# EmilDohne/compressed-image

Hardware: AMD Instinct MI355X
Metric: compress+decompress GB/s (uncompressed side) (higher is better)
Workload: dtype u8

## Files before the change

compressed-image_amd/csrc/encode_kernel.h:

```cpp
#pragma once
#include "codec_types.h"
#include "wave.h"
#include "decode_kernel.h"
#include "blosclz_kernel.h"
#include "zstd_encode.h"
#include "assemble_kernel.h"

namespace cimg {

struct EncodeArgs {
    const ChunkDesc* descs;
    int32_t nchunks;
    CodecParams p;
    const uint8_t* raw;
    uint8_t* scratch;
    StreamRec* recs;
    int32_t lds_bytes;
    int32_t total_blocks;
    int32_t want_split;
    uint64_t* dbg;
    uint32_t* queue;
    int32_t uniform_nblocks;
    int32_t block_items;
    uint32_t* zstd_seq;
    int32_t zstd_seq_stride;
    const ZstdEncTables* zstd_tables;
    uint32_t* queue_next;
    int32_t nwaves;
    int32_t assemble;
    uint8_t* comp;
    ChunkLayout* layout;
    ChunkLayout* layout_host;
    uint32_t* chunk_count;
    uint32_t* ready;
    int32_t* next_item;
    uint32_t gen;
    uint32_t* placed = nullptr;
    int32_t helpers = 0;
};

enum : int { ENC_NQ = 64, ENC_QSTRIDE = 32 };

enum : int { LZ4_HASH_BYTES = 16384, LZ4_MAX_INPUT_U16 = 65536 + 11 - 1 };

inline int encode_lds_bytes(int stream_bytes, int compcode = CODEC_LZ4)
{
    return compcode == CODEC_BLOSCLZ ? blz_encode_lds_bytes(stream_bytes) : round16(stream_bytes) + (compcode == CODEC_ZSTD ? (2 << ZSTD_ENC_HASH_BITS) : LZ4_HASH_BYTES);
}
CIMG_HD int encode_items(int total_blocks, int streams_per_block, bool split, int whole_blocks = 0)
{
    return split ? whole_blocks + (total_blocks - whole_blocks) * streams_per_block : total_blocks;
}
CIMG_HD bool encode_block_items_ok(int typesize, int filter, int blocksize)
{
    return (typesize == 2 || typesize == 4) && filter == FILTER_SHUFFLE && blocksize == 32768;
}

#if defined(CIMG_PROFILE) && !defined(CIMG_EMULATE)
#define CIMG_ITEM_STAMP(dbg, item, k) ((void)0)
#else
#define CIMG_ITEM_STAMP(dbg, item, k) debug_stamp(dbg, item, k)
#endif

#ifdef CIMG_EMULATE
extern long g_emu_windows, g_emu_matches, g_emu_collisions;
#define CIMG_STAT(x) (++(x))
#else
#define CIMG_STAT(x) ((void)0)
#endif

template <int HB = 13>
CIMG_DEV uint32_t lz4_hash(uint32_t v) { return (v * 2654435761u) >> (32 - HB); }
CIMG_DEV int skip_prefix(int n) { const int q = n >> 6, r = n & 63; return q * (32 * (q - 1) + r); }

CIMG_DEV void emit_len_ext(cimg_global_u8p out, int pos, int rem)
{
    const int n255 = rem / 255, last = rem - 255 * n255;
#ifndef CIMG_EMULATE
#pragma unroll 1
#endif
    for (int c = 0; c <= n255; c += 64) {
        FOR_LANES(l) { if (c + l <= n255) out[pos + c + l] = (uint8_t)(c + l < n255 ? 255 : last); }
    }
}

CIMG_DEV void emit_literals(const uint8_t* in, int from, cimg_global_u8p out, int pos, int count)
{
#ifndef CIMG_EMULATE
#pragma unroll 1
#endif
    for (int c = 0; c < count; c += 64) {
        FOR_LANES(l) { if (c + l < count) out[pos + c + l] = in[from + c + l]; }
    }
}

CIMG_DEV int match_more(const uint8_t* in, int ip, int mp, int maxc, int from, int n)
{
    int mcode = from;
    for (int it = 0; it <= n / 256 + 1; ++it) {
        LV<int> len;
        LV<bool> stop;
        FOR_LANES(l) {
            const int k = mcode + 4 * l;
            const uint32_t x = lds_ld32u(in, ip + 4 + k) ^ lds_ld32u(in, mp + 4 + k);
            const int ln = imin(x ? (int)(__builtin_ctz(x) >> 3) : 4, imax(maxc - k, 0));
            len[l] = ln;
            stop[l] = ln < 4;
        }
        const uint64_t sm = ballot(stop);
        if (sm) { const int f = ctz64(sm); return mcode + 4 * f + readlane(len, f); }
        mcode += 256;
    }
    return mcode;
}

CIMG_DEV int div255(int x) { return (int)(((uint64_t)(uint32_t)x * 0x80808081ull) >> 39); }

CIMG_DEV bool emit_pending(const uint8_t* in, cimg_global_u8p out, int cap, int& op, int& need, int np,
                           const LV<int>& P_anchor, const LV<int>& P_lit, const LV<int>& P_off, const LV<int>& P_mcode)
{
    LV<int> size, start, le, me;
    FOR_LANES(l) {
        const int lit = P_lit[l], mc = P_mcode[l];
        le[l] = lit >= 15 ? div255(lit - 15) + 1 : 0;
        me[l] = mc >= 15 ? div255(mc - 15) + 1 : 0;
        size[l] = l < np ? lit + 3 + le[l] + me[l] : 0;
    }
    int total;
    wave_exscan(size, start, total);
    LV<int> lhs, tokpos, litpos;
    LV<bool> fail, ext, shortlit, longlit;
    FOR_LANES(l) {
        const int lit = P_lit[l], mc = P_mcode[l];
        const bool act = l < np;
        tokpos[l] = op + start[l];
        litpos[l] = tokpos[l] + 1 + le[l];
        const int lhs1 = tokpos[l] + 1 + lit + 8 + div255(lit);
        const int lhs2 = litpos[l] + lit + 8 + div255(mc + 240);
        fail[l] = act && (lhs1 > cap || lhs2 > cap);
        lhs[l] = act ? imax(lhs1, lhs2) : 0;
        ext[l] = act && (le[l] > 0 || me[l] > 0);
        shortlit[l] = act && lit > 0 && lit <= 8;
        longlit[l] = act && lit > 8;
    }
    if (ballot(fail)) return false;
    need = imax(need, wave_max(lhs));
    FOR_LANES(l) {
        if (l < np) {
            const int lit = P_lit[l], mc = P_mcode[l], off = P_off[l];
            const int offpos = litpos[l] + lit;
            out[tokpos[l]] = (uint8_t)(((lit >= 15 ? 15 : lit) << 4) | (mc >= 15 ? 15 : mc));
            out[offpos] = (uint8_t)(off & 0xFF);
            out[offpos + 1] = (uint8_t)(off >> 8);
        }
    }
    if (ballot(ext)) {
        for (int r = 0; r < 4; ++r) {
            LV<bool> more;
            FOR_LANES(l) {
                const int lit = P_lit[l], mc = P_mcode[l];
                const bool act = l < np;
                const int le4 = le[l] <= 4 ? le[l] : 0, me4 = me[l] <= 4 ? me[l] : 0;
                if (act && r < le4) out[tokpos[l] + 1 + r] = (uint8_t)(r == le4 - 1 ? lit - 15 - 255 * (le4 - 1) : 255);
                if (act && r < me4) out[litpos[l] + lit + 2 + r] = (uint8_t)(r == me4 - 1 ? mc - 15 - 255 * (me4 - 1) : 255);
                more[l] = act && (r + 1 < le4 || r + 1 < me4);
            }
            if (!ballot(more)) break;
        }
        LV<bool> bigl, bigm;
        FOR_LANES(l) { bigl[l] = l < np && le[l] > 4; bigm[l] = l < np && me[l] > 4; }
        for (uint64_t m = ballot(bigl); m; m &= m - 1) {
            const int k = ctz64(m);
            emit_len_ext(out, readlane(tokpos, k) + 1, readlane(P_lit, k) - 15);
        }
        for (uint64_t m = ballot(bigm); m; m &= m - 1) {
            const int k = ctz64(m);
            emit_len_ext(out, readlane(litpos, k) + readlane(P_lit, k) + 2, readlane(P_mcode, k) - 15);
        }
    }
    if (ballot(shortlit)) {
        for (int r = 0; r < 8; ++r) {
            LV<bool> more;
            FOR_LANES(l) {
                if (shortlit[l] && r < P_lit[l]) out[litpos[l] + r] = in[P_anchor[l] + r];
                more[l] = shortlit[l] && r + 1 < P_lit[l];
            }
            if (!ballot(more)) break;
        }
    }
    uint64_t longm = ballot(longlit);
    while (longm) {
        const int k = ctz64(longm);
        longm &= longm - 1;
        emit_literals(in, readlane(P_anchor, k), out, readlane(litpos, k), readlane(P_lit, k));
    }
    op += total;
    return true;
}

template <int HB = 13>
CIMG_DEV bool lz4_no_match_at_all(const uint8_t* in, cimg_lds_vu16p tab16, int n, int s64, int f64, int mflimit_p1)
{
    bool verdict = false;
    for (int t0 = 0; t0 <= n; t0 += 64) {
        {
            LV<int> p1, p2;
            LV<bool> in2;
            FOR_LANES(l) {
                const int ta = t0 + l, tb = t0 + 64 + l;
                int pa = 1 + ta;
                if (ta > 0) pa = 2 + skip_prefix(s64 + ta - 1) - f64;
                const int pb = 2 + skip_prefix(s64 + tb - 1) - f64, gb = (s64 + tb - 1) >> 6;
                p1[l] = pa; p2[l] = pb;
                in2[l] = pb + gb <= mflimit_p1;
            }
            if (!~ballot(in2)) {
                LV<uint32_t> v1, v2, h1, h2, o1, o2, r1, r2, c1, c2;
                FOR_LANES(l) { v1[l] = lds_ld32u(in, p1[l]); v2[l] = lds_ld32u(in, p2[l]); h1[l] = lz4_hash<HB>(v1[l]); h2[l] = lz4_hash<HB>(v2[l]); }
                FOR_LANES(l) { o1[l] = tab16[h1[l]]; }
                FOR_LANES_W(l) { tab16[h1[l]] = (uint16_t)p1[l]; }
                FOR_LANES(l) { r1[l] = tab16[h1[l]]; }
                FOR_LANES(l) { o2[l] = tab16[h2[l]]; }
                FOR_LANES_W(l) { tab16[h2[l]] = (uint16_t)p2[l]; }
                FOR_LANES(l) { r2[l] = tab16[h2[l]]; c1[l] = lds_ld32u(in, (int)o1[l]); c2[l] = lds_ld32u(in, (int)o2[l]); }
                LV<bool> eventful;
                FOR_LANES(l) {
                    eventful[l] = (r1[l] != (uint32_t)(uint16_t)p1[l]) | (c1[l] == v1[l]) | (r2[l] != (uint32_t)(uint16_t)p2[l]) | (c2[l] == v2[l]);
                }
                if (!ballot(eventful)) { CIMG_STAT(g_emu_windows); CIMG_STAT(g_emu_windows); t0 += 64; continue; }
                FOR_LANES_W(l) { tab16[h2[l]] = (uint16_t)o2[l]; }
                FOR_LANES_W(l) { tab16[h1[l]] = (uint16_t)o1[l]; }
            }
        }
        LV<int> pos;
        LV<bool> inside;
        FOR_LANES(l) {
            const int t = t0 + l;
            int p = 1 + t, gap = 1;
            if (t > 0) { p = 2 + skip_prefix(s64 + t - 1) - f64; gap = (s64 + t - 1) >> 6; }
            pos[l] = p;
            inside[l] = p + gap <= mflimit_p1;
        }
        const uint64_t in_mask = ballot(inside);
        if (!in_mask) { verdict = true; break; }
        LV<uint32_t> v, h, old, rb, cv;
        LV<bool> lost, equal;
        FOR_LANES(l) { v[l] = lds_ld32u(in, inside[l] ? pos[l] : 0); h[l] = lz4_hash<HB>(v[l]); }
        FOR_LANES(l) { old[l] = tab16[h[l]]; }
        FOR_LANES_W(l) { if (inside[l]) tab16[h[l]] = (uint16_t)pos[l]; }
        FOR_LANES(l) { rb[l] = tab16[h[l]]; cv[l] = lds_ld32u(in, (int)old[l]); }
        FOR_LANES(l) {
            lost[l] = inside[l] & (rb[l] != (uint32_t)(uint16_t)pos[l]);
            equal[l] = inside[l] & (cv[l] == v[l]);
        }
        if (ballot(equal)) break;
        if (ballot(lost)) {
            LV<uint32_t> rb2, wv;
            LV<bool> crowd, same;
            FOR_LANES_W(l) { if (lost[l]) tab16[h[l]] = (uint16_t)pos[l]; }
            FOR_LANES(l) { rb2[l] = tab16[h[l]]; wv[l] = lds_ld32u(in, (int)rb[l]); }
            FOR_LANES(l) {
                crowd[l] = lost[l] & (rb2[l] != (uint32_t)(uint16_t)pos[l]);
                same[l] = lost[l] & (wv[l] == v[l]);
            }
            if (ballot(crowd) | ballot(same)) break;
            FOR_LANES_W(l) { if (inside[l] && rb2[l] != (uint32_t)(uint16_t)pos[l] && (uint32_t)pos[l] > rb2[l]) tab16[h[l]] = (uint16_t)pos[l]; }
        }
        CIMG_STAT(g_emu_windows);
        if (~in_mask) { verdict = true; break; }
    }
    return verdict;
}

template <bool SEQ = false>
CIMG_DEV int lz4_encode_body(const uint8_t* in, uint8_t* tab, int n, uint8_t* out_generic, int cap, int accel, int& need_out, uint64_t* dbg = nullptr, int item = 0, SeqSink* sink = nullptr)
{
    constexpr int HB = SEQ ? ZSTD_ENC_HASH_BITS : 13;
    cimg_global_u8p out = CIMG_AS_GLOBAL(out_generic);
    CIMG_PROF_DECL;
    (void)dbg; (void)item;

    cimg_lds_vu16p tab16 = CIMG_AS_LDS_VU16(tab);
    {
        const u128 z = {0, 0, 0, 0};
        for (int u0 = 0; u0 < (2 << HB) / 16; u0 += 64) {
            FOR_LANES(l) { st128a(tab + 16 * (u0 + l), z); }
        }
    }
    const int mflimit_p1 = n - 11, matchlimit = n - 5;
    const int s64 = accel << 6;
    const int f64 = skip_prefix(s64);
    int anchor = 0, op = 0, need = 0;
    LV<int> P_anchor, P_lit, P_off, P_mcode;
    int np = 0;
    FOR_LANES(l) { P_anchor[l] = 0; P_lit[l] = 0; P_off[l] = 0; P_mcode[l] = 0; }

    bool hopeless = false;
    if (n >= 13 + 64) {
        hopeless = lz4_no_match_at_all<HB>(in, tab16, n, s64, f64, mflimit_p1);
        if (hopeless) anchor = 0;
        else {
            const u128 z = {0, 0, 0, 0};
            for (int u0 = 0; u0 < (2 << HB) / 16; u0 += 64) {
                FOR_LANES(l) { st128a(tab + 16 * (u0 + l), z); }
            }
        }
    }
    if (n >= 13 && !hopeless) {
        {
            LV<uint32_t> v0;
            FOR_LANES(l) { v0[l] = lds_ld32u(in, 0); }
            FOR_LANES_W(l) { tab16[lz4_hash<HB>(v0[l])] = 0; }
        }
        CIMG_PROF_LAP(0);
        int sstart = 1;
        int t0 = 0;
        int pre = 0;
        LV<uint32_t> Wn;
        FOR_LANES(l) { Wn[l] = 0; }
        [[maybe_unused]] int chain_credit = 2;
        int guard = 0;
        int ending = 1;
        for (;;) {
            if (++guard > 2 * n + 4) { ending = -1; break; }
            LV<int> pos;
            LV<bool> valid;
            LV<uint32_t> v, h, back;
            int ip = 0, mp = 0, mcode = 0, backrun = 0;
            bool zero_lit = false;
            auto run_path = [&](const uint32_t v0, const uint32_t backv) {
                const int ip0 = sstart - 1;
                const uint32_t h0 = lz4_hash<HB>(v0);
                const uint32_t bbbb = (v0 & 0xFF) * 0x01010101u;
                FOR_LANES_W(l) { tab16[lz4_hash<HB>(backv)] = (uint16_t)(sstart - 3); }
                LV<uint32_t> slot, scan;
                LV<uint32_t> before;
                FOR_LANES(l) {
                    slot[l] = tab16[h0];
                    scan[l] = lds_ld32u(in, ip0 + 5 + 4 * l);
                    before[l] = in[ip0 - 1];
                }
                const int old0 = (int)readlane(slot, 0);
                LV<uint32_t> cw, iw;
                FOR_LANES(l) {
                    cw[l] = lds_ld32u(in, old0 + 4 * l);
                    iw[l] = lds_ld32u(in, ip0 + 4 * l);
                }
                needed_here(scan); needed_here(before); needed_here(iw);
                const bool hit0 = readlane(cw, 0) == v0;
                CIMG_STAT(g_emu_matches);
                if (hit0) {
                    CIMG_PROF_COUNT(5);
                    FOR_LANES_W(l) { tab16[h0] = (uint16_t)ip0; }
                    ip = ip0; mp = old0; zero_lit = true; backrun = 0;
                    const int maxc = matchlimit - (ip0 + 4);
                    LV<int> len;
                    LV<bool> stop;
                    FOR_LANES(l) {
                        const int k = 4 * (l - 1);
                        const uint32_t x = cw[l] ^ iw[l];
                        const int ln = imin(x ? (int)(__builtin_ctz(x) >> 3) : 4, imax(maxc - k, 0));
                        len[l] = ln;
                        stop[l] = (l >= 1) & (ln < 4);
                    }
                    const uint64_t sm = ballot(stop);
                    if (sm) { const int f = ctz64(sm); mcode = 4 * (f - 1) + readlane(len, f); }
                    else mcode = match_more(in, ip0, old0, maxc, 252, n);
                } else {
                    FOR_LANES_W(l) { tab16[h0] = (uint16_t)(ip0 + 1); }
                    ip = ip0 + 1; mp = ip0; zero_lit = false; mcode = 0;
                    backrun = (readlane(before, 0) == (v0 & 0xFF)) ? 1 : 0;
                    const int maxc = matchlimit - (ip + 4);
                    for (int scans = 0; scans <= n / 256 + 2; ++scans) {
                        LV<int> len;
                        LV<bool> stop;
                        FOR_LANES(l) {
                            const int k = mcode + 4 * l;
                            int vb = maxc - k;
                            vb = vb < 0 ? 0 : (vb > 4 ? 4 : vb);
                            int ln = 0;
                            if (vb > 0) {
                                const uint32_t x = scan[l] ^ bbbb;
                                ln = x ? (int)(__builtin_ctz(x) >> 3) : 4;
                                if (ln > vb) ln = vb;
                            }
                            len[l] = ln;
                            stop[l] = ln < 4;
                        }
                        const uint64_t sm = ballot(stop);
                        if (sm) { const int f = ctz64(sm); mcode += 4 * f + readlane(len, f); break; }
                        mcode += 256;
                        FOR_LANES(l) { scan[l] = lds_ld32u(in, ip + 4 + mcode + 4 * l); }
                    }
                }
            };
            const auto sequence = [&](auto extended_tag, int ip, int mp, int mcode, int backrun, const bool zero_lit) -> int {
            if constexpr (!decltype(extended_tag)::value) {
            CIMG_PROF_COUNT(3);
            const int room = zero_lit ? 0 : imin(ip - anchor, mp);
            const int maxc = matchlimit - (ip + 4);
                LV<bool> eq, stop;
                LV<int> len;
                FOR_LANES(l) {
                    const int kb = l < room ? l + 1 : 0;
                    const uint32_t pa = in[ip - kb], pb = in[mp - kb];
                    const int k = 4 * l;
                    const uint32_t x = lds_ld32u(in, ip + 4 + k) ^ lds_ld32u(in, mp + 4 + k);
                    eq[l] = (l < room) & (pa == pb);
                    const int ln = imin(x ? (int)(__builtin_ctz(x) >> 3) : 4, imax(maxc - k, 0));
                    len[l] = ln;
                    stop[l] = ln < 4;
                }
                backrun = ctz64(~ballot(eq));
                const uint64_t sm = ballot(stop);
                if (sm) {
                    const int f = ctz64(sm);
                    mcode = 4 * f + readlane(len, f);
                } else {
                    CIMG_PROF_COUNT(4);
                    mcode = match_more(in, ip, mp, maxc, 256, n);
                }
                if (backrun == 64) {
                    int left = room - 64;
                    while (left > 0) {
                        FOR_LANES(l) { eq[l] = l < left && in[ip - 1 - backrun - l] == in[mp - 1 - backrun - l]; }
                        const int r = ctz64(~ballot(eq));
                        backrun += r; left -= r;
                        if (r < 64) break;
                    }
                }
            }
            CIMG_PROF_LAP(4); CIMG_PROF_COUNT(2);
            ip -= backrun; mp -= backrun; mcode += backrun;
            const int lit = zero_lit ? 0 : ip - anchor;
#ifdef CIMG_ZERO_LIT_CHAIN
            chain_credit = zero_lit ? imin(chain_credit + 3, 8) : imax(chain_credit - (chain_credit > 0 ? 0 : 2), -8);
#endif
            FOR_LANES(l) { Wn[l] = lds_ld32u(in, ip + mcode + 4 - 2 + 4 * (l < 2 ? l : 2)); }
            {
                const int slot = np;
                FOR_LANES(l) {
                    if (l == slot) { P_anchor[l] = anchor; P_lit[l] = lit; P_off[l] = ip - mp; P_mcode[l] = mcode; }
                }
                if (++np == 64) {
                    bool fits_;
                    if constexpr (SEQ) fits_ = zstd_take_parked(in, out, cap, op, *sink, np, P_anchor, P_lit, P_off, P_mcode);
                    else fits_ = emit_pending(in, out, cap, op, need, np, P_anchor, P_lit, P_off, P_mcode);
                    if (!fits_) return 2;
                    np = 0;
                }
            }
            ip += mcode + 4;
            anchor = ip;
            CIMG_PROF_LAP(5);
            if (ip >= mflimit_p1) return 1;
            sstart = ip + 1;
            t0 = 0;
            pre = 1;
            return 0;
            };
#define CIMG_SEQUENCE_IN_HEAD(EXT) { const int r_ = sequence(std::EXT##_type{}, ip, mp, mcode, backrun, zero_lit); if (r_) { if (r_ == 2) ending = 0; stop = true; break; } continue; }
#define CIMG_SEQUENCE(EXT) { const int r_ = sequence(std::EXT##_type{}, ip, mp, mcode, backrun, zero_lit); if (r_) { if (r_ == 2) ending = 0; break; } continue; }
            bool headed = false, stop = false;
            if (pre && t0 == 0 && s64 == 64)
            while (mflimit_p1 - sstart >= 3) {
                if (++guard > 2 * n + 4) { ending = -1; stop = true; break; }
#ifdef CIMG_ZERO_LIT_CHAIN
                if (chain_credit > 0) {
                    int chained = 0;
                    CIMG_PROF_LAP(1);
                    uint32_t cw0 = readlane(Wn, 0), cw1 = readlane(Wn, 1);
                    for (;;) {
                        if (mflimit_p1 - sstart < 3) break;
                        if (++guard > 2 * n + 4) { ending = -1; stop = true; break; }
                        const int ip0 = sstart - 1;
                        const uint32_t v0 = (cw0 >> 16) | (cw1 << 16);
                        const uint32_t h0 = lz4_hash<HB>(v0);
                        FOR_LANES_W(l) { tab16[lz4_hash<HB>(cw0)] = (uint16_t)(sstart - 3); }
                        LV<uint32_t> slot;
                        FOR_LANES(l) { slot[l] = tab16[h0]; }
                        const int c0 = (int)readlane(slot, 0);
                        LV<uint32_t> cw, iw;
                        FOR_LANES(l) {
                            cw[l] = lds_ld32u(in, c0 + 4 * l);
                            iw[l] = lds_ld32u(in, ip0 + 4 * l);
                        }
                        needed_here(cw); needed_here(iw);
                        if (readlane(cw, 0) != v0) { chain_credit -= chained ? 0 : 2; CIMG_PROF_LAP(0); CIMG_PROF_COUNT(4); break; }
                        FOR_LANES_W(l) { tab16[h0] = (uint16_t)ip0; }
                        CIMG_STAT(g_emu_matches);
                        const int maxc = matchlimit - (ip0 + 4);
                        LV<int> len;
                        LV<bool> stopl;
                        FOR_LANES(l) {
                            const int k = 4 * (l - 1);
                            const uint32_t x = cw[l] ^ iw[l];
                            const int ln = imin(x ? (int)(__builtin_ctz(x) >> 3) : 4, imax(maxc - k, 0));
                            len[l] = ln;
                            stopl[l] = (l >= 1) & (ln < 4);
                        }
                        const uint64_t sm = ballot(stopl);
                        int mc;
                        if (sm) { const int f = ctz64(sm); mc = 4 * (f - 1) + readlane(len, f); }
                        else mc = match_more(in, ip0, c0, maxc, 252, n);
                        setlane(P_anchor, np, ip0);
                        setlane(P_lit, np, 0);
                        setlane(P_off, np, ip0 - c0);
                        setlane(P_mcode, np, mc);
                        if (++np == 64) {
                            bool fits_;
                            if constexpr (SEQ) fits_ = zstd_take_parked(in, out, cap, op, *sink, np, P_anchor, P_lit, P_off, P_mcode);
                            else fits_ = emit_pending(in, out, cap, op, need, np, P_anchor, P_lit, P_off, P_mcode);
                            if (!fits_) { ending = 0; stop = true; break; }
                            np = 0;
                        }
                        const int d = mc + 4;
                        CIMG_PROF_LAP(7); CIMG_PROF_COUNT(7);
                        anchor = ip0 + d;
                        chained = 1;
                        chain_credit = imin(chain_credit + 3, 8);
                        if (anchor >= mflimit_p1) { stop = true; break; }
                        sstart = anchor + 1;
                        if (d <= 249) {
                            const int a = (d - 2) >> 2;
                            const uint32_t sh = (uint32_t)(d - 2) & 3u;
                            const uint32_t q0 = readlane(iw, a), q1 = readlane(iw, a + 1), q2 = readlane(iw, a + 2);
                            cw0 = alignbyte(q1, q0, sh);
                            cw1 = alignbyte(q2, q1, sh);
                        } else {
                            LV<uint32_t> far;
                            FOR_LANES(l) { far[l] = lds_ld32u(in, anchor - 2 + 4 * (l < 2 ? l : 2)); }
                            cw0 = readlane(far, 0); cw1 = readlane(far, 1);
                        }
                    }
                    if (stop) break;
                    if (chained) {
                        if (mflimit_p1 - sstart < 3) break;
                        FOR_LANES(l) { Wn[l] = lds_ld32u(in, anchor - 2 + 4 * (l < 2 ? l : 2)); }
                    }
                }
#endif
                const int ip0 = sstart - 1;
                const uint32_t w0 = readlane(Wn, 0), w1 = readlane(Wn, 1);
                const uint32_t v0 = (w0 >> 16) | (w1 << 16), v1 = (w0 >> 24) | (w1 << 8), v2 = w1;
                CIMG_PROF_LAP(1);
                if (v0 == v1) {
                    run_path(v0, w0);
                    CIMG_PROF_LAP(2); CIMG_PROF_COUNT(0);
                    CIMG_SEQUENCE_IN_HEAD(true)
                } else {
                    const uint32_t h0 = lz4_hash<HB>(v0), h1 = lz4_hash<HB>(v1), h2 = lz4_hash<HB>(v2);
                    const int clean = h1 == h0 ? 1 : ((h2 == h0 || h2 == h1) ? 2 : 3);
                    FOR_LANES_W(l) { tab16[lz4_hash<HB>(w0)] = (uint16_t)(sstart - 3); }
                    LV<uint32_t> hl, vl, old3;
                    LV<bool> hit3;
                    FOR_LANES(l) {
                        hl[l] = l == 0 ? h0 : (l == 1 ? h1 : h2);
                        vl[l] = l == 0 ? v0 : (l == 1 ? v1 : v2);
                        old3[l] = tab16[hl[l]];
                    }
                    FOR_LANES(l) { hit3[l] = (l < clean) & (lds_ld32u(in, (int)old3[l]) == vl[l]); }
                    const uint64_t hm = ballot(hit3);
                    if (hm) {
                        const int m3 = ctz64(hm);
                        FOR_LANES_W(l) { if (l <= m3) tab16[hl[l]] = (uint16_t)(ip0 + l); }
                        ip = ip0 + m3;
                        mp = (int)readlane(old3, m3);
                        zero_lit = m3 == 0;
                        CIMG_STAT(g_emu_matches);
                        CIMG_PROF_COUNT(7);
                        CIMG_PROF_LAP(7);
                        CIMG_SEQUENCE_IN_HEAD(false)
                    }
                    CIMG_PROF_LAP(7);
                }
                headed = true;
                break;
            }
            if (stop) break;
            if (headed) {
                const uint32_t w0 = readlane(Wn, 0), w1 = readlane(Wn, 1);
                const uint32_t v0 = (w0 >> 16) | (w1 << 16), v1 = (w0 >> 24) | (w1 << 8), v2 = w1;
                const uint32_t h0 = lz4_hash<HB>(v0), h1 = lz4_hash<HB>(v1), h2 = lz4_hash<HB>(v2);
                const bool e21 = h2 == h1;
                if ((e21 && v2 == v1) || (!e21 && h2 == h0 && v2 == v0)) {
                    const int p0 = sstart - 1;
                    FOR_LANES_W(l) { tab16[h0] = (uint16_t)p0; }
                    FOR_LANES_W(l) { tab16[h1] = (uint16_t)(p0 + 1); }
                    FOR_LANES_W(l) { tab16[h2] = (uint16_t)(p0 + 2); }
                    ip = p0 + 2;
                    mp = e21 ? p0 + 1 : p0;
                    zero_lit = false;
                    CIMG_STAT(g_emu_matches);
                    CIMG_SEQUENCE(false)
                }
            }
            const int backpos = pre ? sstart - 3 : 0;
            const bool dense = t0 == 0 && s64 == 64;
            int nv = 64;
            if (dense) {
                const int first = sstart - pre;
                nv = imin(64, pre + imax(mflimit_p1 - sstart, 0));
                FOR_LANES(l) {
                    pos[l] = first + l;
                    valid[l] = l < nv;
                    v[l] = lds_ld32u(in, l < nv ? first + l : 0);
                    h[l] = lz4_hash<HB>(v[l]);
                    back[l] = lds_ld32u(in, backpos);
                }
// ... 837 lines not shown
```

Measured before the change: 631.3.

## Add bulk distinct-value proof to skip LZ4 no-match emulation on noise chunks

Adds an optional pre-pass that samples the chunk's 4-byte values at the positions the LZ4 skip schedule would probe and checks them for duplicates using multi-round hashed LDS tables. If all values are proven distinct, the chunk is marked hopeless without running the sequential no-match emulation. Otherwise it falls back to that emulation, reusing the prefilter work for the first window. The path only compiles under CIMG_BULK_NOMATCH and adds LDS traffic and register pressure when the proof fails.

```diff
diff --git a/compressed-image_amd/csrc/encode_kernel.h b/compressed-image_amd/csrc/encode_kernel.h
--- a/compressed-image_amd/csrc/encode_kernel.h
+++ b/compressed-image_amd/csrc/encode_kernel.h
@@ -199,11 +199,11 @@
 }
 
 template <int HB = 13>
-CIMG_DEV bool lz4_no_match_at_all(const uint8_t* in, cimg_lds_vu16p tab16, int n, int s64, int f64, int mflimit_p1)
+CIMG_DEV bool lz4_no_match_at_all(const uint8_t* in, cimg_lds_vu16p tab16, int n, int s64, int f64, int mflimit_p1, bool first_double_done = false)
 {
     bool verdict = false;
     for (int t0 = 0; t0 <= n; t0 += 64) {
-        {
+        if (!(first_double_done && t0 == 0)) {
             LV<int> p1, p2;
             LV<bool> in2;
             FOR_LANES(l) {
@@ -272,6 +272,269 @@
     return verdict;
 }
 
+template <int HB>
+CIMG_DEV void lz4_clear_table(uint8_t* tab)
+{
+    const u128 z = {0, 0, 0, 0};
+    for (int u0 = 0; u0 < (2 << HB) / 16; u0 += 64) {
+        FOR_LANES(l) { st128a(tab + 16 * (u0 + l), z); }
+    }
+}
+
+#if defined(CIMG_BULK_NOMATCH) && !defined(CIMG_NO_BULK_NOMATCH)
+enum : int { NOISE_PREFILTER = 0, NOISE_DISTINCT = 1, NOISE_MAYBE = 2, NOISE_ROUNDS = 8 };
+#ifdef CIMG_EMULATE
+inline long g_emu_noise_path[3] = {0, 0, 0};
+inline long g_emu_noise_rounds = 0;
+#endif
+
+template <int HB>
+CIMG_DEV uint32_t noise_hash(uint32_t v, int shift) { return ((v * 2654435761u) >> shift) & ((1u << HB) - 1u); }
+#ifdef CIMG_EMULATE
+CIMG_DEV int noise_mul24(int a, int b) { return a * b; }
+#else
+CIMG_DEV int noise_mul24(int a, int b) { return __mul24(a, b); }
+#endif
+CIMG_DEV int noise_member_pos(int r, int l, int accel, int c0)
+{
+    const int q = accel + r;
+    const int p = c0 + noise_mul24(q, 32 * (q - 1) + l);
+    return r == 63 ? l : p;
+}
+
+CIMG_DEV uint32_t noise_ld32u(cimg_lds_cu8p lds, int off)
+{
+    const int a = off & ~3;
+    const uint32_t lo = *CIMG_AS_LDS_CU32(lds + a);
+    const uint32_t hi = *CIMG_AS_LDS_CU32(lds + a + 4);
+    return alignbyte(hi, lo, (uint32_t)off & 3u);
+}
+
+template <int HB, int G>
+CIMG_DEV void noise_rows_write(cimg_lds_cu8p in, cimg_lds_vu16p tab16, int r0, int accel, int c0, int shift)
+{
+    LV<int> pos[G];
+    LV<uint32_t> h[G];
+    CIMG_UNROLL
+    for (int g = 0; g < G; ++g) {
+        const int q = accel + r0 + g, base = c0 + 32 * q * (q - 1);
+        FOR_LANES(l) { pos[g][l] = base + noise_mul24(q, l); }
+    }
+    CIMG_UNROLL
+    for (int g = 0; g < G; ++g) {
+        FOR_LANES(l) { h[g][l] = noise_hash<HB>(noise_ld32u(in, pos[g][l]), shift); }
+    }
+    CIMG_UNROLL
+    for (int g = 0; g < G; ++g) {
+        FOR_LANES_W(l) { tab16[h[g][l]] = (uint16_t)pos[g][l]; }
+    }
+}
+template <int HB, int G>
+CIMG_DEV void noise_rows_read(cimg_lds_cu8p in, cimg_lds_vu16p tab16, int r0, int accel, int c0, int shift, LV<uint64_t>& lose, LV<bool>& equal)
+{
+    LV<int> pos[G];
+    LV<uint32_t> v[G], h[G], rb[G], cv[G];
+    CIMG_UNROLL
+    for (int g = 0; g < G; ++g) {
+        const int q = accel + r0 + g, base = c0 + 32 * q * (q - 1);
+        FOR_LANES(l) { pos[g][l] = base + noise_mul24(q, l); }
+    }
+    CIMG_UNROLL
+    for (int g = 0; g < G; ++g) {
+        FOR_LANES(l) { v[g][l] = noise_ld32u(in, pos[g][l]); h[g][l] = noise_hash<HB>(v[g][l], shift); }
+    }
+    CIMG_UNROLL
+    for (int g = 0; g < G; ++g) {
+        FOR_LANES(l) { rb[g][l] = tab16[h[g][l]]; }
+    }
+    CIMG_UNROLL
+    for (int g = 0; g < G; ++g) {
+        FOR_LANES(l) { cv[g][l] = noise_ld32u(in, (int)rb[g][l]); }
+    }
+    CIMG_UNROLL
+    for (int g = 0; g < G; ++g) {
+        const uint64_t bit = 1ull << (r0 + g);
+        FOR_LANES(l) {
+            const bool lost = rb[g][l] != (uint32_t)(uint16_t)pos[g][l];
+            equal[l] = equal[l] | (lost & (cv[g][l] == v[g][l]));
+            lose[l] |= lost ? bit : 0ull;
+        }
+    }
+}
+enum : int { NOISE_VROWS = 4 };
+template <int HB>
+CIMG_DEV void noise_vrows_write(cimg_lds_cu8p in, cimg_lds_vu16p tab16, LV<uint64_t>& w, int accel, int c0, int shift)
+{
+    constexpr int G = NOISE_VROWS;
+    LV<int> pos[G];
+    LV<bool> act[G];
+    LV<uint32_t> h[G];
+    CIMG_UNROLL
+    for (int g = 0; g < G; ++g) {
+        FOR_LANES(l) {
+            act[g][l] = w[l] != 0;
+            const int p = noise_member_pos(ctz64(w[l]) & 63, l, accel, c0);
+            pos[g][l] = act[g][l] ? p : 0;
+            w[l] &= w[l] - 1;
+        }
+    }
+    CIMG_UNROLL
+    for (int g = 0; g < G; ++g) {
+        FOR_LANES(l) { h[g][l] = noise_hash<HB>(noise_ld32u(in, pos[g][l]), shift); }
+    }
+    CIMG_UNROLL
+    for (int g = 0; g < G; ++g) {
+        FOR_LANES_W(l) { if (act[g][l]) tab16[h[g][l]] = (uint16_t)pos[g][l]; }
+    }
+}
+template <int HB>
+CIMG_DEV void noise_vrows_read(cimg_lds_cu8p in, cimg_lds_vu16p tab16, LV<uint64_t>& w, int accel, int c0, int shift, LV<uint64_t>& lose, LV<bool>& equal)
+{
+    constexpr int G = NOISE_VROWS;
+    LV<int> pos[G];
+    LV<uint64_t> bit[G];
+    LV<bool> act[G];
+    LV<uint32_t> v[G], h[G], rb[G], cv[G];
+    CIMG_UNROLL
+    for (int g = 0; g < G; ++g) {
+        FOR_LANES(l) {
+            act[g][l] = w[l] != 0;
+            const int p = noise_member_pos(ctz64(w[l]) & 63, l, accel, c0);
+            pos[g][l] = act[g][l] ? p : 0;
+            bit[g][l] = w[l] & (0 - w[l]);
+            w[l] &= w[l] - 1;
+        }
+    }
+    CIMG_UNROLL
+    for (int g = 0; g < G; ++g) {
+        FOR_LANES(l) { v[g][l] = noise_ld32u(in, pos[g][l]); h[g][l] = noise_hash<HB>(v[g][l], shift); }
+    }
+    CIMG_UNROLL
+    for (int g = 0; g < G; ++g) {
+        FOR_LANES(l) { rb[g][l] = tab16[h[g][l]]; }
+    }
+    CIMG_UNROLL
+    for (int g = 0; g < G; ++g) {
+        FOR_LANES(l) {
+            act[g][l] = act[g][l] & (rb[g][l] != (uint32_t)(uint16_t)pos[g][l]);
+            cv[g][l] = noise_ld32u(in, act[g][l] ? (int)rb[g][l] : 0);
+        }
+    }
+    CIMG_UNROLL
+    for (int g = 0; g < G; ++g) {
+        FOR_LANES(l) {
+            equal[l] = equal[l] | (act[g][l] & (cv[g][l] == v[g][l]));
+            lose[l] |= act[g][l] ? bit[g][l] : 0ull;
+        }
+    }
+}
+
+template <int HB = 13>
+CIMG_DEV_OUTLINE int lz4_probe_values_distinct(cimg_lds_cu8p in, cimg_lds_vu16p tab16, int n, int s64, int f64, int mflimit_p1)
+{
+    (void)n;
+    {
+        LV<int> p1, p2;
+        LV<bool> in2;
+        FOR_LANES(l) {
+            const int tb = 64 + l;
+            int pa = 1 + l;
+            if (l > 0) pa = 2 + skip_prefix(s64 + l - 1) - f64;
+            const int pb = 2 + skip_prefix(s64 + tb - 1) - f64, gb = (s64 + tb - 1) >> 6;
+            p1[l] = pa; p2[l] = pb;
+            in2[l] = pb + gb <= mflimit_p1;
+        }
+        if (!~ballot(in2)) {
+            LV<uint32_t> v1, v2, h1, h2, o1, o2, c1, c2;
+            FOR_LANES(l) { v1[l] = noise_ld32u(in, p1[l]); v2[l] = noise_ld32u(in, p2[l]); h1[l] = lz4_hash<HB>(v1[l]); h2[l] = lz4_hash<HB>(v2[l]); }
+            FOR_LANES(l) { o1[l] = tab16[h1[l]]; }
+            FOR_LANES_W(l) { tab16[h1[l]] = (uint16_t)p1[l]; }
+            FOR_LANES(l) { o2[l] = tab16[h2[l]]; }
+            FOR_LANES_W(l) { tab16[h2[l]] = (uint16_t)p2[l]; }
+            FOR_LANES(l) { c1[l] = noise_ld32u(in, (int)o1[l]); c2[l] = noise_ld32u(in, (int)o2[l]); }
+            LV<bool> equal;
+            FOR_LANES(l) { equal[l] = (c1[l] == v1[l]) | (c2[l] == v2[l]); }
+            if (ballot(equal)) {
+                FOR_LANES_W(l) { tab16[h2[l]] = (uint16_t)o2[l]; }
+                FOR_LANES_W(l) { tab16[h1[l]] = (uint16_t)o1[l]; }
+                CIMG_STAT(g_emu_noise_path[NOISE_PREFILTER]);
+                return NOISE_PREFILTER;
+            }
+        }
+    }
+    const int accel = s64 >> 6, c0 = 2 - f64;
+    int full = 0;
+    if (accel <= 1024) {
+        for (; full < 62; ++full) {
+            const int q = accel + full;
+            if (c0 + q * (32 * (q - 1) + 63) + q > mflimit_p1) break;
+        }
+    }
+    if (accel > 1024 || full >= 62) { CIMG_STAT(g_emu_noise_path[NOISE_MAYBE]); return NOISE_MAYBE; }
+    LV<uint64_t> part;
+    FOR_LANES(l) {
+        const bool partial = noise_member_pos(full, l, accel, c0) + accel + full <= mflimit_p1;
+        part[l] = (partial ? 1ull << full : 0ull) | (l < 2 ? 1ull << 63 : 0ull);
+    }
+    int verdict = NOISE_MAYBE;
+#ifdef CIMG_EMULATE
+    g_emu_noise_rounds = 0;
+#endif
+    for (int k = 0; k < NOISE_ROUNDS; ++k) {
+        CIMG_STAT(g_emu_noise_rounds);
+        const int shift = (32 - HB) - (int)((0x5C83A6D0u >> (4 * k)) & 15u);
+        LV<uint64_t> w, lose;
+        LV<bool> equal;
+        if (k == 0) {
+            int r = 0;
+#ifndef CIMG_EMULATE
+#pragma unroll 1
+#endif
+            for (; r + 8 <= full; r += 8) noise_rows_write<HB, 8>(in, tab16, r, accel, c0, shift);
+            if (r + 4 <= full) { noise_rows_write<HB, 4>(in, tab16, r, accel, c0, shift); r += 4; }
+            if (r + 2 <= full) { noise_rows_write<HB, 2>(in, tab16, r, accel, c0, shift); r += 2; }
+            if (r < full) noise_rows_write<HB, 1>(in, tab16, r, accel, c0, shift);
+        }
+        FOR_LANES(l) { w[l] = part[l]; }
+#ifndef CIMG_EMULATE
+#pragma unroll 1
+#endif
+        for (int j = 0; j < 64; j += NOISE_VROWS) {
+            LV<bool> any;
+            FOR_LANES(l) { any[l] = w[l] != 0; }
+            if (!ballot(any)) break;
+            noise_vrows_write<HB>(in, tab16, w, accel, c0, shift);
+        }
+        FOR_LANES(l) { w[l] = part[l]; lose[l] = 0; equal[l] = false; }
+        if (k == 0) {
+            int r = 0;
+#ifndef CIMG_EMULATE
+#pragma unroll 1
+#endif
+            for (; r + 8 <= full; r += 8) noise_rows_read<HB, 8>(in, tab16, r, accel, c0, shift, lose, equal);
+            if (r + 4 <= full) { noise_rows_read<HB, 4>(in, tab16, r, accel, c0, shift, lose, equal); r += 4; }
+            if (r + 2 <= full) { noise_rows_read<HB, 2>(in, tab16, r, accel, c0, shift, lose, equal); r += 2; }
+            if (r < full) noise_rows_read<HB, 1>(in, tab16, r, accel, c0, shift, lose, equal);
+        }
+#ifndef CIMG_EMULATE
+#pragma unroll 1
+#endif
+        for (int j = 0; j < 64; j += NOISE_VROWS) {
+            LV<bool> any;
+            FOR_LANES(l) { any[l] = w[l] != 0; }
+            if (!ballot(any)) break;
+            noise_vrows_read<HB>(in, tab16, w, accel, c0, shift, lose, equal);
+        }
+        if (ballot(equal)) break;
+        LV<bool> some;
+        FOR_LANES(l) { some[l] = lose[l] != 0; part[l] = lose[l]; }
+        if (!ballot(some)) { verdict = NOISE_DISTINCT; break; }
+    }
+    CIMG_STAT(g_emu_noise_path[verdict]);
+    return verdict;
+}
+#endif
+
 template <bool SEQ = false>
 CIMG_DEV int lz4_encode_body(const uint8_t* in, uint8_t* tab, int n, uint8_t* out_generic, int cap, int accel, int& need_out, uint64_t* dbg = nullptr, int item = 0, SeqSink* sink = nullptr)
 {
@@ -297,14 +560,18 @@
 
     bool hopeless = false;
     if (n >= 13 + 64) {
+#if defined(CIMG_BULK_NOMATCH) && !defined(CIMG_NO_BULK_NOMATCH)
+        const int proof = lz4_probe_values_distinct<HB>(CIMG_AS_LDS_CU8(in), tab16, n, s64, f64, mflimit_p1);
+        if (proof == NOISE_DISTINCT) hopeless = true;
+        else {
+            if (proof == NOISE_MAYBE) lz4_clear_table<HB>(tab);
+            hopeless = lz4_no_match_at_all<HB>(in, tab16, n, s64, f64, mflimit_p1, proof == NOISE_PREFILTER);
+        }
+#else
         hopeless = lz4_no_match_at_all<HB>(in, tab16, n, s64, f64, mflimit_p1);
+#endif
         if (hopeless) anchor = 0;
-        else {
-            const u128 z = {0, 0, 0, 0};
-            for (int u0 = 0; u0 < (2 << HB) / 16; u0 += 64) {
-                FOR_LANES(l) { st128a(tab + 16 * (u0 + l), z); }
-            }
-        }
+        else lz4_clear_table<HB>(tab);
     }
     if (n >= 13 && !hopeless) {
         {
```

After: 624.7. -1.1%, worse.
